# adamjorr/kbbq

Measured on AMD Instinct MI355X. Metric: recalibrated Gbases/sec, higher is better.
Workload: dtype u64

## Files before the change

kbbq_amd/csrc/engine.hip:

```cpp
#include <hip/hip_runtime.h>

#include <algorithm>
#include <cstdarg>
#include <cstdio>
#include <cstdlib>
#include <cstring>
#include <map>
#include <mutex>
#include <string>
#include <thread>
#include <vector>

#include "../../include/kbbq_engine.h"
#include "abi_internal.h"
#include "correct.h"
#include "correct_wave.h"
#include "device_common.h"
#include "host_model.h"

using namespace kbbq;

static thread_local char g_err[512] = "";
int kbbq_fail(int code, const char *fmt, ...) {
    va_list ap;
// ... 11 lines not shown
                        hipGetErrorString(_e), __FILE__, __LINE__);                                    \
    } while (0)

#include "kernels.h"
#include "bucket.h"
#include "long_reads.h"


struct FilterHost {
    FilterSpec spec;
    uint64_t *d_table = nullptr;
    uint64_t *d_patterns = nullptr;
    unsigned long long *d_inserted = nullptr;
    uint64_t table_bytes() const { return spec.n_blocks * kEngineBlockBytes; }
    FiltDev dev() const {
        FiltDev f;
        f.table = reinterpret_cast<ulonglong2 *>(d_table);
        f.patterns = reinterpret_cast<const ulonglong2 *>(d_patterns);
        f.n_blocks = spec.n_blocks;
        const ModMagic mm = make_mod_magic(spec.n_blocks);
        f.mod_magic = mm.m64;
        f.mod_m32 = mm.m32;
        f.salt0 = spec.salt[0];
        f.salt1 = spec.salt[1];
        return f;
    }
};

struct ProfileSlot {
    std::string name;
    uint64_t launches = 0;
    double ms = 0;
};
struct PendingEvent {
    int slot;
    hipEvent_t a, b;
};

struct Options {
    bool no_overlap = false;
    bool no_fastpath = false;
    bool lane_walk = false;
    bool no_pass4_pipeline = false;
    int pass2_side = 2;
    bool tally_general = false;
    bool infer_subset = true;
    bool debug_bucket = false;
    int bucket = -1;
    uint64_t bucket_records = 0;
    uint64_t pass4_piece = 0;
    int scan_blocks = -1;
    int walk_blocks = -1;
    int infer_blocks = 0;
};

struct kbbq_engine {
    kbbq_params p;
    Options opt;
    KParams K;
    hipStream_t stream = nullptr;
    hipStream_t stream2 = nullptr;
    hipEvent_t ev_main = nullptr, ev_side[2] = {nullptr, nullptr};
    hipEvent_t ev_draw = nullptr, ev_ins[2] = {nullptr, nullptr};
    bool ins_pending[2] = {false, false};
    int draw_turn = 0;
    bool side_busy[2] = {false, false};
    bool pass3_shared = false;
    unsigned long long *d_totals = nullptr;
    int side_turn = 0;
    uint32_t *d_qpresent = nullptr;
    uint32_t qpresent[8] = {};
    bool qpresent_known = false;
    uint8_t *d_dq_qslot = nullptr;
    int dq_slots = 0;
    uint32_t *d_rg_present[2] = {nullptr, nullptr};
    hipStream_t cur = nullptr;
    unsigned long long *cur_cnt = nullptr;
    FilterHost filt[2];
    Xoshiro256 seed_state;
    uint64_t draw_threshold = 0;
    bool draw_always = false;
    bool thresholds_set = false;
    std::vector<int32_t> thresholds;
    unsigned long long *d_hist = nullptr;
    uint64_t hist_cycle_words = 0, hist_dinuc_words = 0;
    DqTables dq;
    bool dq_set = false;
    int16_t *d_dq_base = nullptr;
    int8_t *d_dq_cycle = nullptr;
    int8_t *d_dq_dinuc = nullptr;
    void *scratch[24] = {};
    size_t scratch_bytes[24] = {};
    unsigned long long *d_counters = nullptr;
    unsigned int *d_tickets = nullptr;
    struct StageSlot {
        char *dev = nullptr;
        size_t bytes = 0;
        hipEvent_t h2d = nullptr, done[2] = {nullptr, nullptr};
        hipEvent_t d2h = nullptr;
        bool busy[2] = {false, false};
        bool d2h_pending = false;
        uint32_t gen = 0;
    } slot[3];
    int slot_turn = 0, cur_slot = -1;
    bool cur_slot_side = false;
    bool cur_h2d_recorded = false;
    bool async_call = false;
    uint64_t last_ticket = 0;
    hipStream_t copy = nullptr;
    uint64_t stats[4] = {0, 0, 0, 0};
    std::vector<ProfileSlot> prof;
    std::vector<PendingEvent> pending;
    uint32_t *d_qcum = nullptr, *d_errthr = nullptr;
    uint32_t qcum_len = 0;
    struct Buckets {
        int mode[2] = {-1, -1};
        bool allocated = false;
        uint64_t capacity = 0;
        void *l1 = nullptr, *l2 = nullptr;
        uint32_t *l1_cnt = nullptr, *l2_cnt = nullptr, *tickets = nullptr;
        unsigned long long *direct = nullptr;
        bool pending[2] = {false, false};
        double pending_est[2] = {0, 0};
        double frac_trusted = 0.75;
        double frac_used = 0.75;
        uint64_t bases_since[2] = {0, 0}, inserted_at_flush[2] = {0, 0};
        uint64_t flushes[2] = {0, 0};
        hipStream_t stream[2] = {nullptr, nullptr};
        hipEvent_t ev_flush = nullptr;
        unsigned long long *h_inserted = nullptr;
        hipEvent_t ev_est = nullptr;
        bool est_pending = false, est_known = false;
        uint64_t est_bases = 0, est_prev = 0, cur_bases = 0;
    } bk;
    hipEvent_t ev_infer = nullptr, ev_take[2] = {nullptr, nullptr};
    bool take_pending[2] = {false, false};
    int take_turn = 0;
    size_t attr_lds_tally = 0, attr_lds_recal = 0;
    std::map<const void *, size_t> attr_lds_correct;
};

namespace {

int ensure_scratch(kbbq_engine *e, int idx, size_t bytes) {
    if (e->scratch_bytes[idx] >= bytes) return KBBQ_OK;
    if (e->scratch[idx]) {
        HIP_TRY(hipStreamSynchronize(e->stream));
        HIP_TRY(hipStreamSynchronize(e->stream2));
        HIP_TRY(hipFree(e->scratch[idx]));
        e->scratch[idx] = nullptr;
        e->scratch_bytes[idx] = 0;
    }
    const size_t want = bytes + bytes / 8 + 256;
    HIP_TRY(hipMalloc(&e->scratch[idx], want));
    e->scratch_bytes[idx] = want;
    return KBBQ_OK;
}

static void plan_tally_slots(TallyPlan &P, const uint32_t mask[8], int max_slots, int n_rg) {
    memset(P.qslot, 255, sizeof P.qslot);
    memset(P.qof, 0, sizeof P.qof);
    P.n_slots = 0;
    max_slots = std::max(1, std::min(max_slots, 255));
    int top = -1, distinct = 0;
    for (int q = 0; q < KBBQ_NQ; ++q)
        if ((mask[q >> 5] >> (q & 31)) & 1) { top = q; ++distinct; }
    if (top >= 0 && top + 1 <= max_slots && (n_rg <= 1 || 2 * distinct >= top + 1)) {
        for (int q = 0; q <= top; ++q) { P.qof[q] = (uint8_t)q; P.qslot[q] = (uint8_t)q; }
        P.n_slots = top + 1;
        P.identity = 1;
    } else {
        for (int q = 0; q < KBBQ_NQ && P.n_slots < max_slots; ++q)
            if ((mask[q >> 5] >> (q & 31)) & 1) { P.qof[P.n_slots] = (uint8_t)q; P.qslot[q] = (uint8_t)P.n_slots++; }
        P.identity = 0;
    }
    if (P.n_slots == 0) { P.n_slots = 1; P.qof[0] = 0; P.qslot[0] = 0; P.identity = 1; }
    P.rg_base = 0; P.n_rgs = 1; P.cbase = 0; P.direct_cycles = 0;
}

struct Timed {
    kbbq_engine *e;
    int slot = -1;
    hipEvent_t a = nullptr, b = nullptr;
    hipStream_t on = nullptr;
    Timed(kbbq_engine *e_, const char *name, hipStream_t stream = nullptr) : e(e_), on(stream ? stream : e_->stream) {
        if (!(e->p.flags & KBBQ_F_PROFILE)) return;
        for (size_t i = 0; i < e->prof.size(); ++i)
            if (e->prof[i].name == name) slot = (int)i;
        if (slot < 0) {
            ProfileSlot s;
            s.name = name;
            e->prof.push_back(s);
            slot = (int)e->prof.size() - 1;
        }
        hipEventCreate(&a);
        hipEventCreate(&b);
        hipEventRecord(a, on);
    }
    ~Timed() {
        if (slot < 0) return;
        hipEventRecord(b, on);
        PendingEvent pe = {slot, a, b};
        e->pending.push_back(pe);
    }
};

void drain_profile(kbbq_engine *e) {
    for (size_t i = 0; i < e->pending.size(); ++i) {
        PendingEvent &pe = e->pending[i];
        float ms = 0;
        if (hipEventSynchronize(pe.b) == hipSuccess && hipEventElapsedTime(&ms, pe.a, pe.b) == hipSuccess) {
            e->prof[pe.slot].ms += ms;
            e->prof[pe.slot].launches += 1;
        }
        hipEventDestroy(pe.a);
        hipEventDestroy(pe.b);
    }
    e->pending.clear();
}

__global__ void k_add_counters(const unsigned long long *side, const unsigned long long *offcase, unsigned long long *totals) {
    totals[0] += side[0] + offcase[0];
    totals[1] += side[1];
}

int collect_totals(kbbq_engine *e) {
    unsigned long long t[2] = {0, 0};
    HIP_TRY(hipMemcpy(t, e->d_totals, 16, hipMemcpyDeviceToHost));
    e->stats[0] = t[0];
    e->stats[1] = t[1];
    e->side_busy[0] = e->side_busy[1] = false;
    return KBBQ_OK;
}

int sync_engine(kbbq_engine *e) {
    HIP_TRY(hipStreamSynchronize(e->stream));
    HIP_TRY(hipStreamSynchronize(e->stream2));
    if (e->side_busy[0] || e->side_busy[1]) {
        int rc = collect_totals(e);
        if (rc) return rc;
    }
    drain_profile(e);
    return KBBQ_OK;
}

struct HostBatchDone {
    kbbq_engine *e;
    HostBatchDone(kbbq_engine *e_, const kbbq_reads *) : e(e_) { e->cur_slot = -1; e->cur_slot_side = false; e->cur_h2d_recorded = false; e->last_ticket = 0; }
    ~HostBatchDone() {
        if (e->cur_slot < 0) return;
        kbbq_engine::StageSlot &s = e->slot[e->cur_slot];
        if (hipEventRecord(s.done[0], e->stream) == hipSuccess) s.busy[0] = true;
        if (e->cur_slot_side && hipEventRecord(s.done[1], e->stream2) == hipSuccess) s.busy[1] = true;
        if (e->async_call && e->cur_h2d_recorded) {
            e->last_ticket = ((uint64_t)s.gen << 8) | (uint64_t)(e->cur_slot + 1);
        } else if (e->cur_h2d_recorded) {
            hipEventSynchronize(s.h2d);
        } else {
            hipStreamSynchronize(e->copy);
        }
        e->cur_slot = -1;
    }
};

typedef KbbqDeviceGuard DeviceGuard;
#define ENGINE_DEVICE(e)                                                                              \
    if (!(e)) return fail(KBBQ_EINVAL, "null engine");                                                \
    DeviceGuard engine_device_guard((e)->p.device);                                                   \
    if (engine_device_guard.err != hipSuccess)                                                        \
        return fail(KBBQ_EIO, "hipSetDevice(%d): %s", (e)->p.device, hipGetErrorString(engine_device_guard.err))

hipStream_t shared_copy_stream(int device) {
    static std::mutex m;
    static std::map<int, hipStream_t> streams;
    std::lock_guard<std::mutex> lock(m);
    std::map<int, hipStream_t>::iterator it = streams.find(device);
    if (it != streams.end()) return it->second;
    hipStream_t st = nullptr;
    if (hipStreamCreateWithFlags(&st, hipStreamNonBlocking) != hipSuccess) return nullptr;
    streams[device] = st;
    return st;
}

int acquire_slot(kbbq_engine *e, size_t need, kbbq_engine::StageSlot **out) {
    kbbq_engine::StageSlot &s = e->slot[e->slot_turn];
    for (int t = 0; t < 2; ++t)
        if (s.busy[t]) { HIP_TRY(hipEventSynchronize(s.done[t])); s.busy[t] = false; }
    if (s.d2h_pending) { HIP_TRY(hipEventSynchronize(s.d2h)); s.d2h_pending = false; }
    s.gen += 1;
    if (s.bytes < need) {
// ... 328 lines not shown
    int rc = bucket_flush(e, 1 - w);
    if (rc) return rc;
    b.cur_bases = bases;
    if (b.pending[w] && b.pending_est[w] + est > 0.93 * (double)b.capacity) {
        if ((rc = bucket_flush(e, w, false))) return rc;
        if (w == 1) est = (est - 4096.0) / std::max(1e-9, b.frac_used) * b.frac_trusted + 4096.0;
    }
    b.cur_bases = 0;
    b.pending[w] = true;
    b.pending_est[w] += est;
    b.bases_since[w] += bases;
    return KBBQ_OK;
}

}


extern "C" {

const char *kbbq_last_error(void) { return g_err; }

int kbbq_engine_create(const kbbq_params *params, kbbq_engine **out) {
    if (!params || !out) return fail(KBBQ_EINVAL, "null argument");
    if (params->k < 1 || params->k > KBBQ_MAX_KMER) return fail(KBBQ_ERANGE, "k must be <= %d and > 0", KBBQ_MAX_KMER);
    if (params->n_rg < 1 || params->n_rg > 65535) return fail(KBBQ_EINVAL, "n_rg must be in 1..65535");
    if (params->max_read_len < 1 || params->max_read_len > KBBQ_MAX_READ_LEN)
        return fail(KBBQ_ERANGE, "max_read_len must be in 1..%d", KBBQ_MAX_READ_LEN);
    int ndev = 0;
    if (hipGetDeviceCount(&ndev) != hipSuccess || ndev == 0) return fail(KBBQ_ENODEV, "no HIP device visible");
    if (params->device < 0 || params->device >= ndev) return fail(KBBQ_ENODEV, "device %d of %d", params->device, ndev);
    DeviceGuard create_guard(params->device);
    HIP_TRY(create_guard.err);
    kbbq_engine *e = new kbbq_engine;
    e->p = *params;
    {
        Options &o = e->opt;
        auto env_set = [](const char *name) { const char *v = getenv(name); return v && *v; };
        auto env_int = [](const char *name, int dflt) { const char *v = getenv(name); return v && *v ? atoi(v) : dflt; };
        const int fl = params->flags;
        o.no_overlap = (fl & KBBQ_F_NO_OVERLAP) || env_set("KBBQ_NO_OVERLAP");
        o.no_fastpath = (fl & KBBQ_F_NO_FASTPATH) || env_set("KBBQ_NO_FASTPATH");
        o.lane_walk = (fl & KBBQ_F_LANE_WALK) || (getenv("KBBQ_CORRECT") && !strcmp(getenv("KBBQ_CORRECT"), "lane"));
        o.no_pass4_pipeline = (fl & KBBQ_F_NO_PASS4_PIPELINE) || env_set("KBBQ_NO_PASS4_PIPELINE");
        o.pass2_side = (fl & KBBQ_F_PASS2_INORDER) ? 0 : env_int("KBBQ_PASS2_SIDE", o.pass2_side);
        o.tally_general = env_set("KBBQ_TALLY_GENERAL");
        o.infer_subset = env_int("KBBQ_INFER_SUBSET", 1) != 0;
        o.debug_bucket = env_set("KBBQ_DEBUG_BUCKET");
        o.bucket = (fl & KBBQ_F_BUCKET_ON) ? 1 : (fl & KBBQ_F_BUCKET_OFF) ? 0 : env_set("KBBQ_BUCKET") ? (env_int("KBBQ_BUCKET", 0) != 0 ? 1 : 0) : -1;
        o.bucket_records = env_u64("KBBQ_BUCKET_RECORDS", 0);
        o.pass4_piece = env_u64("KBBQ_PASS4_PIECE", 0);
        o.scan_blocks = env_int("KBBQ_SCAN_BLOCKS", o.scan_blocks);
        o.walk_blocks = env_int("KBBQ_WALK_BLOCKS", o.walk_blocks);
        o.infer_blocks = env_int("KBBQ_INFER_BLOCKS", o.infer_blocks);
    }
    e->K.k = params->k;
    e->K.shift = 2u * (unsigned)(params->k - 1);
    e->K.mask = params->k < 32 ? ((1ULL << (2 * params->k)) - 1) : ~0ULL;
    e->K.nmask_bits = params->k < 32 ? ((1u << params->k) - 1) : 0xFFFFFFFFu;
    const double fprs[2] = {params->fpr_sampled, params->fpr_trusted};
    for (int w = 0; w < 2; ++w) {
        if (!make_filter_spec(params->approx_kmers, fprs[w], params->bloom_seed, e->filt[w].spec)) {
            delete e;
            return fail(KBBQ_EINVAL, "Error: Invalid bloom filter parameters. Adjust parameters and try again.");
        }
    }
    hipError_t he = hipStreamCreateWithFlags(&e->stream, hipStreamNonBlocking);
    if (he == hipSuccess) he = hipStreamCreateWithFlags(&e->stream2, hipStreamNonBlocking);
    if (he == hipSuccess) he = hipEventCreateWithFlags(&e->ev_main, hipEventDisableTiming);
    if (he == hipSuccess) he = hipEventCreateWithFlags(&e->ev_draw, hipEventDisableTiming);
    for (int t = 0; t < 2 && he == hipSuccess; ++t) he = hipEventCreateWithFlags(&e->ev_ins[t], hipEventDisableTiming);
    if (he == hipSuccess) he = hipEventCreateWithFlags(&e->ev_side[0], hipEventDisableTiming);
    if (he == hipSuccess) he = hipEventCreateWithFlags(&e->ev_side[1], hipEventDisableTiming);
    if (he == hipSuccess) he = hipStreamCreateWithFlags(&e->copy, hipStreamNonBlocking);
    if (he == hipSuccess) he = hipEventCreateWithFlags(&e->bk.ev_flush, hipEventDisableTiming);
    if (he == hipSuccess) he = hipEventCreateWithFlags(&e->bk.ev_est, hipEventDisableTiming);
    if (he == hipSuccess) he = hipEventCreateWithFlags(&e->ev_infer, hipEventDisableTiming);
    for (int t = 0; t < 2 && he == hipSuccess; ++t) he = hipEventCreateWithFlags(&e->ev_take[t], hipEventDisableTiming);
    if (he == hipSuccess) he = hipHostMalloc((void **)&e->bk.h_inserted, 64, hipHostMallocDefault);
    for (int i = 0; i < 3 && he == hipSuccess; ++i) {
        he = hipEventCreateWithFlags(&e->slot[i].h2d, hipEventDisableTiming);
        if (he == hipSuccess) he = hipEventCreateWithFlags(&e->slot[i].d2h, hipEventDisableTiming);
        for (int t = 0; t < 2 && he == hipSuccess; ++t) he = hipEventCreateWithFlags(&e->slot[i].done[t], hipEventDisableTiming);
    }
    e->cur = e->stream;
    if (he != hipSuccess) { kbbq_engine_destroy(e); return fail(KBBQ_EIO, "hipStreamCreate: %s", hipGetErrorString(he)); }
#define CREATE_TRY(expr)                                                                           \
    do {                                                                                           \
        hipError_t _e = (expr);                                                                    \
        if (_e != hipSuccess) {                                                                    \
            int code = _e == hipErrorOutOfMemory ? KBBQ_ENOMEM : KBBQ_EIO;                         \
            fail(code, "%s: %s", #expr, hipGetErrorString(_e));                                    \
            kbbq_engine_destroy(e);                                                                \
            return code;                                                                           \
        }                                                                                          \
    } while (0)
    CREATE_TRY(hipMalloc(&e->d_counters, 64));
    CREATE_TRY(hipMemset(e->d_counters, 0, 64));
    CREATE_TRY(hipMalloc(&e->d_tickets, 64));
    CREATE_TRY(hipMemset(e->d_tickets, 0, 64));
    CREATE_TRY(hipMalloc(&e->d_totals, 32));
    CREATE_TRY(hipMemset(e->d_totals, 0, 32));
    e->cur_cnt = e->d_counters;
    CREATE_TRY(hipMalloc(&e->d_dq_qslot, KBBQ_NQ));
    CREATE_TRY(hipMalloc(&e->d_qpresent, 32));
    for (int i = 0; i < 2; ++i) CREATE_TRY(hipMalloc(&e->d_rg_present[i], (((size_t)params->n_rg + 31) / 32) * 4 + 4));
    for (int w = 0; w < 2; ++w) {
        FilterHost &f = e->filt[w];
        CREATE_TRY(hipMalloc(&f.d_table, f.table_bytes()));
        CREATE_TRY(hipMalloc(&f.d_patterns, kNumPatterns * kEngineBlockBytes));
        CREATE_TRY(hipMalloc(&f.d_inserted, 8));
        std::vector<uint64_t> packed(kNumPatterns * 2);
        for (uint64_t i = 0; i < kNumPatterns; ++i) {
            if (!squeeze_block(&f.spec.patterns[i * 8], &packed[i * 2])) {
                kbbq_engine_destroy(e);
                return fail(KBBQ_ESTATE, "pattern %llu uses a bit outside the 128 the generator can reach", (unsigned long long)i);
            }
        }
        CREATE_TRY(hipMemcpy(f.d_patterns, packed.data(), kNumPatterns * kEngineBlockBytes, hipMemcpyHostToDevice));
    }
    e->hist_cycle_words = (uint64_t)params->n_rg * kNQ * 2 * params->max_read_len * 2;
    e->hist_dinuc_words = (uint64_t)params->n_rg * kNQ * 16 * 2;
    CREATE_TRY(hipMalloc(&e->d_hist, (e->hist_cycle_words + e->hist_dinuc_words) * 8));
    CREATE_TRY(hipMalloc(&e->d_dq_base, (size_t)params->n_rg * kNQ * 2));
    CREATE_TRY(hipMalloc(&e->d_dq_cycle, (size_t)params->n_rg * kNQ * 2 * params->max_read_len));
    CREATE_TRY(hipMalloc(&e->d_dq_dinuc, (size_t)params->n_rg * kNQ * 16));
    CREATE_TRY(hipMemcpyToSymbol(HIP_SYMBOL(c_jump), xoshiro_jump_table(), 64 * 4 * 8));
    e->seed_state.seed32(params->seed);
    e->draw_threshold = bernoulli_threshold(params->alpha, &e->draw_always);
    int rc = kbbq_engine_reset(e);
    if (rc) { kbbq_engine_destroy(e); return rc; }
    CREATE_TRY(hipDeviceSynchronize());
    *out = e;
    return KBBQ_OK;
}

void kbbq_engine_destroy(kbbq_engine *e) {
    if (!e) return;
    DeviceGuard destroy_guard(e->p.device);
    if (e->stream) { hipStreamSynchronize(e->stream); }
    if (e->stream2) hipStreamSynchronize(e->stream2);
    if (e->copy) hipStreamSynchronize(e->copy);
    drain_profile(e);
    for (int i = 0; i < 3; ++i) {
        hipFree(e->slot[i].dev);
        if (e->slot[i].h2d) hipEventDestroy(e->slot[i].h2d);
        if (e->slot[i].d2h) hipEventDestroy(e->slot[i].d2h);
        for (int t = 0; t < 2; ++t) if (e->slot[i].done[t]) hipEventDestroy(e->slot[i].done[t]);
    }
    if (e->copy) hipStreamDestroy(e->copy);
    if (e->bk.ev_flush) hipEventDestroy(e->bk.ev_flush);
    if (e->bk.ev_est) hipEventDestroy(e->bk.ev_est);
    if (e->ev_infer) hipEventDestroy(e->ev_infer);
    for (int t = 0; t < 2; ++t) if (e->ev_take[t]) hipEventDestroy(e->ev_take[t]);
    if (e->bk.h_inserted) hipHostFree(e->bk.h_inserted);
    for (int w = 0; w < 2; ++w) {
        hipFree(e->filt[w].d_table);
        hipFree(e->filt[w].d_patterns);
        hipFree(e->filt[w].d_inserted);
    }
    hipFree(e->d_hist);
    hipFree(e->d_dq_base);
    hipFree(e->d_dq_cycle);
    hipFree(e->d_dq_dinuc);
    hipFree(e->d_counters);
    hipFree(e->d_tickets);
    hipFree(e->d_totals);
    hipFree(e->d_dq_qslot);
    hipFree(e->d_qpresent);
    hipFree(e->d_rg_present[0]);
    hipFree(e->d_rg_present[1]);
    hipFree(e->d_qcum);
    hipFree(e->d_errthr);
    hipFree(e->bk.l1); hipFree(e->bk.l2); hipFree(e->bk.l1_cnt); hipFree(e->bk.l2_cnt); hipFree(e->bk.tickets); hipFree(e->bk.direct);
    for (int i = 0; i < 24; ++i) hipFree(e->scratch[i]);
    if (e->stream2) { hipStreamSynchronize(e->stream2); hipStreamDestroy(e->stream2); }
    if (e->ev_main) hipEventDestroy(e->ev_main);
    if (e->ev_draw) hipEventDestroy(e->ev_draw);
    for (int t = 0; t < 2; ++t) if (e->ev_ins[t]) hipEventDestroy(e->ev_ins[t]);
    for (int i = 0; i < 2; ++i) if (e->ev_side[i]) hipEventDestroy(e->ev_side[i]);
    if (e->stream) hipStreamDestroy(e->stream);
    delete e;
}

int kbbq_engine_reset(kbbq_engine *e) {
    ENGINE_DEVICE(e);
    if (!e) return fail(KBBQ_EINVAL, "null engine");
    int rc0 = sync_engine(e);
    if (rc0) return rc0;
    for (int w = 0; w < 2; ++w) {
        HIP_TRY(hipMemsetAsync(e->filt[w].d_table, 0, e->filt[w].table_bytes(), e->stream));
        HIP_TRY(hipMemsetAsync(e->filt[w].d_inserted, 0, 8, e->stream));
    }
    HIP_TRY(hipMemsetAsync(e->d_hist, 0, (e->hist_cycle_words + e->hist_dinuc_words) * 8, e->stream));
    HIP_TRY(hipMemsetAsync(e->d_counters, 0, 64, e->stream));
    HIP_TRY(hipMemsetAsync(e->d_totals, 0, 16, e->stream));
    HIP_TRY(hipMemsetAsync(e->d_qpresent, 0, 32, e->stream));
    memset(e->qpresent, 0, sizeof e->qpresent);
    e->qpresent_known = false;
    if (e->bk.allocated) {
        HIP_TRY(hipMemsetAsync(e->bk.l1_cnt, 0, kL1CntBytes, e->stream));
        HIP_TRY(hipMemsetAsync(e->bk.l2_cnt, 0, kL2CntBytes, e->stream));
        HIP_TRY(hipMemsetAsync(e->bk.direct, 0, 8, e->stream));
    }
    e->bk.est_pending = false;
    e->bk.est_known = false;
    e->bk.frac_trusted = 0.75;
    e->bk.stream[0] = e->bk.stream[1] = nullptr;
    for (int w = 0; w < 2; ++w) { e->bk.pending[w] = false; e->bk.pending_est[w] = 0; e->bk.bases_since[w] = 0; e->bk.inserted_at_flush[w] = 0; e->bk.flushes[w] = 0; }
    e->thresholds_set = false;
    e->dq_set = false;
    memset(e->stats, 0, sizeof e->stats);
    return sync_engine(e);
}

int kbbq_engine_sync(kbbq_engine *e) {
    ENGINE_DEVICE(e);
    { int frc = bucket_flush_all(e); if (frc) return frc; }
    if (!e) return fail(KBBQ_EINVAL, "null engine");
    return sync_engine(e);
}

void *kbbq_engine_stream(kbbq_engine *e) { return e ? (void *)e->stream : nullptr; }

int kbbq_engine_dims(kbbq_engine *e, uint64_t *n_rg, uint64_t *n_cycle) {
    if (!e) return fail(KBBQ_EINVAL, "null engine");
    if (n_rg) *n_rg = (uint64_t)e->p.n_rg;
    if (n_cycle) *n_cycle = (uint64_t)e->p.max_read_len;
    return KBBQ_OK;
}

int kbbq_engine_tune(kbbq_engine *e, const char *name, uint64_t value) {
    if (!e || !name) return fail(KBBQ_EINVAL, "null argument");
    if (!strcmp(name, "bucket_records")) {
        if (e->bk.allocated) return fail(KBBQ_ESTATE, "the record buffers are allocated already");
        e->opt.bucket_records = value;
    } else if (!strcmp(name, "pass4_piece")) {
        e->opt.pass4_piece = value;
    } else if (!strcmp(name, "scan_blocks") || !strcmp(name, "walk_blocks") || !strcmp(name, "infer_blocks")) {
        if (value > 17) return fail(KBBQ_EINVAL, "%s: 0 (as many as fit) to 16 workgroups per CU, 17 = default", name);
        (name[0] == 's' ? e->opt.scan_blocks : name[0] == 'w' ? e->opt.walk_blocks : e->opt.infer_blocks) = value == 17 ? (name[0] == 'i' ? 0 : -1) : (int)value;
    } else if (!strcmp(name, "infer_subset")) {
        e->opt.infer_subset = value != 0;
    } else if (!strcmp(name, "pass2_side")) {
        ENGINE_DEVICE(e);
        { int frc = bucket_flush_all(e); if (frc) return frc; }
        int rc = sync_engine(e);
        if (rc) return rc;
        if (value > 2) return fail(KBBQ_EINVAL, "pass2_side: 0, 1 or 2");
        e->opt.pass2_side = (int)value;
        e->bk.stream[0] = e->bk.stream[1] = nullptr;
    } else if (!strcmp(name, "no_overlap")) {
        ENGINE_DEVICE(e);
        { int frc = bucket_flush_all(e); if (frc) return frc; }
        int rc = sync_engine(e);
        if (rc) return rc;
        e->opt.no_overlap = value != 0;
        e->bk.stream[0] = e->bk.stream[1] = nullptr;
    } else {
        return fail(KBBQ_EINVAL, "unknown knob '%s'", name);
    }
    return KBBQ_OK;
}

int kbbq_filter_info_get(kbbq_engine *e, int which, kbbq_filter_info *out) {
    ENGINE_DEVICE(e);
    { int frc = bucket_flush_all(e); if (frc) return frc; }
    if (!e || !out || which < 0 || which > 1) return fail(KBBQ_EINVAL, "bad argument");
    const FilterSpec &s = e->filt[which].spec;
    memset(out, 0, sizeof *out);
    out->bits = s.bits;
    out->bits_unblocked = s.bits_unblocked;
    out->n_blocks = s.n_blocks;
    out->table_bytes = e->filt[which].table_bytes();
    out->random_seed = s.random_seed;
    out->n_hash = s.n_hash;
    out->n_salt = s.n_salt;
    for (uint32_t i = 0; i < s.n_salt; ++i) out->salt[i] = s.salt[i];
    int rc = sync_engine(e);
    if (rc) return rc;
    HIP_TRY(hipMemcpy(&out->inserted, e->filt[which].d_inserted, 8, hipMemcpyDeviceToHost));
    return KBBQ_OK;
}

void *kbbq_filter_device_table(kbbq_engine *e, int which) {
    if (!e || which < 0 || which > 1) return nullptr;
    DeviceGuard guard(e->p.device);
    if (guard.err != hipSuccess || bucket_flush_all(e) != KBBQ_OK) return nullptr;
    return e->filt[which].d_table;
}
void *kbbq_filter_device_counter(kbbq_engine *e, int which) { return e && which >= 0 && which < 2 ? e->filt[which].d_inserted : nullptr; }

int kbbq_filter_download(kbbq_engine *e, int which, uint64_t *host_words, uint64_t n_words) {
    ENGINE_DEVICE(e);
// ... 786 lines not shown
        const int dyn_len = ((max_len + 31) / 32) * 32;
        const size_t words = (size_t)C::words_for(dyn_len);
        const uint64_t fit = std::max<uint64_t>(1, ((uint64_t)1 << 30) / (words * 4 * BLOCK));
        const int blocks = (int)std::min<uint64_t>(std::min<uint64_t>((R.n_reads + BLOCK - 1) / BLOCK, 256 * 4), fit);
        const int slot = side ? 21 : 20;
        int rc = ensure_scratch(e, slot, (size_t)blocks * BLOCK * words * 4);
        if (rc) return rc;
        Timed t(e, "k_correct_long", e->cur);
        hipLaunchKernelGGL((k_correct<MAXL, BLOCK>), dim3(blocks), dim3(BLOCK), 0, e->cur, R, e->K, e->filt[1].dev(), list,
                           n_list, tmask, tw, err_bits, patch, e->cur_cnt, dyn_len, (uint32_t *)e->scratch[slot]);
        HIP_TRY(hipGetLastError());
        return KBBQ_OK;
    }
    const size_t lds = (size_t)C::WORDS * BLOCK * 4;
    size_t &raised = e->attr_lds_correct[(const void *)k_correct<MAXL, BLOCK>];
    if (lds > raised) {
        HIP_TRY(hipFuncSetAttribute((const void *)k_correct<MAXL, BLOCK>, hipFuncAttributeMaxDynamicSharedMemorySize, (int)lds));
        raised = lds;
    }
    Timed t(e, "k_correct", e->cur);
    const int blocks = (int)std::min<uint64_t>((R.n_reads + BLOCK - 1) / BLOCK, 256 * 8);
    hipLaunchKernelGGL((k_correct<MAXL, BLOCK>), dim3(blocks), dim3(BLOCK), lds, e->cur, R, e->K, e->filt[1].dev(), list,
                       n_list, tmask, tw, err_bits, patch, e->cur_cnt, 0, (uint32_t *)nullptr);
    HIP_TRY(hipGetLastError());
    return KBBQ_OK;
}

template <int NB, int NN>
static int launch_correct_wave(kbbq_engine *e, ReadsDev R, const uint32_t *list, const uint64_t *tmask, int tw,
                               uint32_t *err_bits, uint32_t *patch) {
    unsigned int *ticket = e->d_tickets + 3 + (e->cur_cnt != e->d_counters ? 1 : 0);
    HIP_TRY(hipMemsetAsync(ticket, 0, 4, e->cur));
    Timed t(e, "k_correct_wave", e->cur);
    const int blocks = wave_grid(R.n_reads, e->pass3_shared ? shared_cap(e, e->opt.walk_blocks, 2, NB <= 5 ? 160 : 512, !R.offsets) : 0);
    hipLaunchKernelGGL((k_correct_wave<NB, NN>), dim3(blocks), dim3(256), 0, e->cur, R, e->K, e->filt[1].dev(), list,
                       (const unsigned long long *)e->cur_cnt, tmask, tw, err_bits, patch, e->cur_cnt, ticket);
    HIP_TRY(hipGetLastError());
    return KBBQ_OK;
}
extern "C" {

static int build_read_index(kbbq_engine *e, const ReadsDev &R, int slot, hipStream_t stream, const uint32_t **index) {
    *index = nullptr;
    if (!R.offsets || !R.n_reads) return KBBQ_OK;
    const size_t entries = R.n_bases / READ_INDEX_STEP + 2;
    int rc = ensure_scratch(e, slot, entries * 4);
    if (rc) return rc;
    hipLaunchKernelGGL(k_read_index, dim3((unsigned)((R.n_reads + 255) / 256)), dim3(256), 0, stream, R.offsets, R.n_reads, (uint32_t *)e->scratch[slot]);
    HIP_TRY(hipGetLastError());
    *index = (const uint32_t *)e->scratch[slot];
    return KBBQ_OK;
}

static int run_tally(kbbq_engine *e, const ReadsDev &R, const uint32_t *err_bits, const uint32_t *patch, int max_len,
                     hipStream_t stream = nullptr) {
    if (!stream) stream = e->cur;
    HistDev H;
    H.cycle = e->d_hist;
    H.dinuc = e->d_hist + e->hist_cycle_words;
    H.n_rg = e->p.n_rg;
    H.n_cycle = e->p.max_read_len;
    const int n_rg = R.rg ? e->p.n_rg : 1;
    const int ccap = std::min(((max_len + 31) / 32) * 32, 192);
    if (!e->qpresent_known) {
        hipLaunchKernelGGL(k_qpresence, dim3(1024), dim3(256), 0, stream, R.qual, R.n_bases, e->d_qpresent);
        HIP_TRY(hipGetLastError());
        HIP_TRY(hipMemcpyAsync(e->qpresent, e->d_qpresent, 32, hipMemcpyDeviceToHost, stream));
        HIP_TRY(hipStreamSynchronize(stream));
    }
    const int n_windows = (max_len + ccap - 1) / ccap;
    const bool direct_cycles = n_windows > kTallyMaxWindows;
    const size_t per_slot = (direct_cycles ? 0 : (size_t)8 * ccap) + 128;
    TallyPlan P;
    plan_tally_slots(P, e->qpresent, (int)((152 * 1024 - 512) / per_slot), n_rg);
    P.direct_cycles = direct_cycles ? 1 : 0;
    const size_t per_rg = (size_t)P.n_slots * per_slot;
    const size_t budget = (size_t)n_rg * per_rg <= 70 * 1024 ? 70 * 1024 : 140 * 1024;
    const int per_launch = (int)std::max<size_t>(1, std::min<size_t>((size_t)n_rg, budget / per_rg));
    const size_t lds = (size_t)per_launch * per_rg + 4 + 256 + 4;
    if (lds > e->attr_lds_tally) {
        HIP_TRY(hipFuncSetAttribute((const void *)k_tally, hipFuncAttributeMaxDynamicSharedMemorySize, (int)lds));
        HIP_TRY(hipFuncSetAttribute((const void *)k_tally_uniform<true>, hipFuncAttributeMaxDynamicSharedMemorySize, (int)lds));
        HIP_TRY(hipFuncSetAttribute((const void *)k_tally_uniform<false>, hipFuncAttributeMaxDynamicSharedMemorySize, (int)lds));
        e->attr_lds_tally = lds;
    }
    const uint64_t groups = (R.n_bases + 15) / 16;
    const int blocks = (int)std::min<uint64_t>((groups + 1023) / 1024, lds <= 76 * 1024 ? 512 : 256);
    const int vec_ok = ((uintptr_t)R.qual & 15) == 0;
    const uint32_t *read_index;
    int rc = build_read_index(e, R, stream == e->stream2 ? 15 : 14, stream, &read_index);
    if (rc) return rc;
    const uint32_t *present = nullptr;
    if (n_rg > per_launch) {
        uint32_t *pr = e->d_rg_present[stream == e->stream2 ? 1 : 0];
        HIP_TRY(hipMemsetAsync(pr, 0, (((size_t)e->p.n_rg + 31) / 32) * 4, stream));
        hipLaunchKernelGGL(k_rg_presence, dim3((unsigned)((R.n_reads + 255) / 256)), dim3(256), 0, stream, R.rg, R.n_reads, (uint32_t)e->p.n_rg, pr);
        present = pr;
    }
    if (!e->opt.tally_general && !R.offsets && n_rg == 1 && n_windows == 1 && R.read_len >= 16 && (int)R.read_len <= ccap && R.n_bases < (1ULL << 32) && vec_ok &&
        e->p.n_rg == 1) {
        const unsigned long long inv_len = ~0ULL / R.read_len + 1;
        Timed t(e, "k_tally", stream);
        if (P.identity) hipLaunchKernelGGL(k_tally_uniform<false>, dim3(blocks), dim3(1024), lds, stream, R, H, err_bits, patch, ccap, 6, inv_len, P);
        else hipLaunchKernelGGL(k_tally_uniform<true>, dim3(blocks), dim3(1024), lds, stream, R, H, err_bits, patch, ccap, 6, inv_len, P);
        HIP_TRY(hipGetLastError());
        return KBBQ_OK;
    }
    Timed t(e, "k_tally", stream);
    for (int g = 0; g < n_rg; g += per_launch)
        for (int w = 0; w < (direct_cycles ? 1 : n_windows); ++w) {
            P.rg_base = g;
            P.n_rgs = std::min(per_launch, n_rg - g);
            P.cbase = w * ccap;
            hipLaunchKernelGGL(k_tally, dim3(blocks), dim3(1024), lds, stream, R, H, err_bits, patch, ccap, 6, vec_ok, P, present, read_index);
        }
    HIP_TRY(hipGetLastError());
    return KBBQ_OK;
}

int kbbq_errors_batch(kbbq_engine *e, const kbbq_reads *reads, uint64_t *errors_out) {
    ENGINE_DEVICE(e);
    { int frc = bucket_flush_all(e); if (frc) return frc; }
    if (!e || !reads) return fail(KBBQ_EINVAL, "null argument");
    const bool own_err = !(errors_out && reads->on_device);
    const bool overlap = own_err && !(errors_out && !reads->on_device) && !e->opt.no_overlap;
    int side = 0, rc;
    if (overlap) {
        side = e->side_turn;
        e->side_turn ^= 1;
        if (e->side_busy[side]) HIP_TRY(hipStreamWaitEvent(e->stream, e->ev_side[side], 0));
    } else {
        if ((rc = sync_engine(e))) return rc;
    }
    e->pass3_shared = overlap;
    HostBatchDone host_done(e, reads);
    ReadsDev R; int max_len;
    if ((rc = device_view(e, reads, &R, &max_len))) return rc;
    const bool long_reads = max_len > kStagedMax;
    const int NW = max_len <= 192 ? 3 : max_len <= 320 ? 5 : !long_reads ? 8 : 8 * ((std::max(1, max_len - e->p.k + 1) + 511) / 512);
    const int s_tmask = side ? 10 : 3, s_dirty = side ? 11 : 4, s_list = side ? 12 : 5, s_err = side ? 8 : 6, s_patch = side ? 9 : 7;
    if ((rc = ensure_scratch(e, s_tmask, R.n_reads * NW * 8))) return rc;
    if ((rc = ensure_scratch(e, s_dirty, R.n_reads))) return rc;
    if ((rc = ensure_scratch(e, s_list, R.n_reads * 4))) return rc;
    if ((rc = ensure_scratch(e, s_patch, R.n_reads * 4))) return rc;
    uint32_t *d_err;
    if (own_err) {
        if ((rc = ensure_scratch(e, s_err, (R.n_bases / 64 + 2) * 8))) return rc;
        d_err = (uint32_t *)e->scratch[s_err];
    } else {
        d_err = (uint32_t *)errors_out;
    }
    e->cur = e->stream;
    e->cur_cnt = e->d_counters + 4 * side;
    struct Restore { kbbq_engine *e; ~Restore() { e->cur = e->stream; e->cur_cnt = e->d_counters; } } restore = {e};
    HIP_TRY(hipMemsetAsync(d_err, 0, (R.n_bases / 64 + 1) * 8, e->cur));
    HIP_TRY(hipMemsetAsync(e->scratch[s_patch], 0, R.n_reads * 4, e->cur));
    HIP_TRY(hipMemsetAsync(e->cur_cnt, 0, 16, e->cur));
    uint64_t *tmask = (uint64_t *)e->scratch[s_tmask];
    uint8_t *dirty = (uint8_t *)e->scratch[s_dirty];
    uint32_t *list = (uint32_t *)e->scratch[s_list];
    uint32_t *patch = (uint32_t *)e->scratch[s_patch];
    const bool no_fast = e->opt.no_fastpath;
    if (long_reads) {
        Timed t(e, "k_scan_trusted_long", e->cur);
        hipLaunchKernelGGL(k_scan_trusted_long, dim3(wave_grid(R.n_reads)), dim3(256), 0, e->cur, R, e->K, e->filt[1].dev(), tmask, NW, dirty);
        HIP_TRY(hipGetLastError());
    } else if ((rc = dispatch_nw<LaunchScan>(max_len, e, R, tmask, dirty, d_err, (!no_fast && e->p.k >= 3) ? 1 : 0, max_len))) return rc;
    {
        Timed t(e, "k_compact", e->cur);
        hipLaunchKernelGGL(k_compact, dim3((unsigned)((R.n_reads + 1023) / 1024)), dim3(1024), 0, e->cur, dirty, R.n_reads, list, e->cur_cnt,
                           long_reads ? 0 : 1);
        HIP_TRY(hipGetLastError());
    }
    if (overlap) {
        HIP_TRY(hipEventRecord(e->ev_main, e->stream));
        HIP_TRY(hipStreamWaitEvent(e->stream2, e->ev_main, 0));
        e->cur = e->stream2;
        e->cur_slot_side = true;
    }
    const bool lane_form = e->opt.lane_walk;
    if (long_reads) {
        rc = launch_correct<0, 64>(e, R, list, e->cur_cnt, tmask, NW, d_err, patch, max_len, side);
    } else if (lane_form || e->p.k < 3) {
        if (max_len <= 160) rc = launch_correct<160, 256>(e, R, list, e->cur_cnt, tmask, NW, d_err, patch);
        else if (max_len <= 320) rc = launch_correct<320, 128>(e, R, list, e->cur_cnt, tmask, NW, d_err, patch);
        else rc = launch_correct<512, 64>(e, R, list, e->cur_cnt, tmask, NW, d_err, patch);
    } else {
        if (max_len <= 160) rc = launch_correct_wave<5, 3>(e, R, list, tmask, NW, d_err, patch);
        else if (max_len <= 320) rc = launch_correct_wave<10, 5>(e, R, list, tmask, NW, d_err, patch);
        else rc = launch_correct_wave<16, 8>(e, R, list, tmask, NW, d_err, patch);
    }
    if (rc) return rc;
    if (R.offcase && !long_reads) {
        if ((rc = ensure_scratch(e, side ? 18 : 17, R.n_reads * 4))) return rc;
        uint32_t *list3 = (uint32_t *)e->scratch[side ? 18 : 17];
        unsigned long long *cnt3 = e->d_counters + 6 + side;
        HIP_TRY(hipMemsetAsync(cnt3, 0, 8, e->cur));
        hipLaunchKernelGGL(k_compact, dim3((unsigned)((R.n_reads + 1023) / 1024)), dim3(1024), 0, e->cur, dirty, R.n_reads, list3, cnt3, 3);
        HIP_TRY(hipGetLastError());
        if (max_len <= 160) rc = launch_correct<160, 256>(e, R, list3, cnt3, tmask, NW, d_err, patch);
        else if (max_len <= 320) rc = launch_correct<320, 128>(e, R, list3, cnt3, tmask, NW, d_err, patch);
        else rc = launch_correct<512, 64>(e, R, list3, cnt3, tmask, NW, d_err, patch);
        if (rc) return rc;
    }
    if ((rc = run_tally(e, R, d_err, patch, max_len, e->cur))) return rc;
    if (!(R.offcase && !long_reads)) HIP_TRY(hipMemsetAsync(e->d_counters + 6 + side, 0, 8, e->cur));
    hipLaunchKernelGGL(k_add_counters, dim3(1), dim3(1), 0, e->cur, (const unsigned long long *)(e->d_counters + 4 * side),
                       (const unsigned long long *)(e->d_counters + 6 + side), e->d_totals);
    HIP_TRY(hipGetLastError());
    HIP_TRY(hipEventRecord(e->ev_side[side], e->cur));
    e->side_busy[side] = true;
    e->stats[2] += R.n_reads;
    if (!overlap) {
        if ((rc = sync_engine(e))) return rc;
        if (errors_out && !reads->on_device)
            HIP_TRY(hipMemcpy(errors_out, d_err, (R.n_bases / 64 + 1) * 8, hipMemcpyDeviceToHost));
    }
    return KBBQ_OK;
}

int kbbq_tally_batch(kbbq_engine *e, const kbbq_reads *reads, const uint64_t *errors) {
    ENGINE_DEVICE(e);
    { int frc = bucket_flush_all(e); if (frc) return frc; }
    if (!e || !errors) return fail(KBBQ_EINVAL, "null argument");
    HostBatchDone host_done(e, reads);
    ReadsDev R; int max_len;
    int rc = device_view(e, reads, &R, &max_len);
    if (rc) return rc;
    const uint32_t *d_err = (const uint32_t *)errors;
    if (!reads->on_device) {
        const size_t bytes = (reads->n_bases / 64 + 1) * 8;
        if ((rc = ensure_scratch(e, 16, bytes + 8))) return rc;
        HIP_TRY(hipMemsetAsync((char *)e->scratch[16] + bytes, 0, 8, e->stream));
        HIP_TRY(hipMemcpyAsync(e->scratch[16], errors, bytes, hipMemcpyHostToDevice, e->stream));
        d_err = (const uint32_t *)e->scratch[16];
    }
    if ((rc = run_tally(e, R, d_err, nullptr, max_len))) return rc;
    return reads->on_device ? KBBQ_OK : sync_engine(e);
}

void *kbbq_covariates_device(kbbq_engine *e, uint64_t *n_words) {
    if (!e) return nullptr;
    if (n_words) *n_words = e->hist_cycle_words + e->hist_dinuc_words;
    return e->d_hist;
}

static int fetch_hist(kbbq_engine *e, std::vector<uint64_t> &cyc, std::vector<uint64_t> &di) {
    int rc = sync_engine(e);
    if (rc) return rc;
    cyc.resize(e->hist_cycle_words);
    di.resize(e->hist_dinuc_words);
    HIP_TRY(hipMemcpy(cyc.data(), e->d_hist, e->hist_cycle_words * 8, hipMemcpyDeviceToHost));
    HIP_TRY(hipMemcpy(di.data(), e->d_hist + e->hist_cycle_words, e->hist_dinuc_words * 8, hipMemcpyDeviceToHost));
    return KBBQ_OK;
}

int kbbq_covariates_get(kbbq_engine *e, kbbq_covariates *out) {
    ENGINE_DEVICE(e);
// ... 408 lines not shown
```

kbbq_amd/csrc/kernels.h:

```cpp
#pragma once
#include <hip/hip_runtime.h>

#include "../../include/kbbq_engine.h"
#include "correct.h"
#include "correct_wave.h"
#include "device_common.h"

using namespace kbbq;


constexpr int DRAWS_PER_LANE = 4096;

__constant__ uint64_t c_jump[64][4];

__device__ __forceinline__ uint64_t xo_next(uint64_t (&s)[4]) {
    uint64_t x = s[1] * 5;
    x = (x << 7) | (x >> 57);
    x *= 9;
    const uint64_t t = s[1] << 17;
    s[2] ^= s[0];
    s[3] ^= s[1];
    s[1] ^= s[2];
    s[0] ^= s[3];
    s[2] ^= t;
// ... 886 lines not shown
                        count(lr, rg, q, second, cyc, (int)((ew >> i) & 1), cyc >= 1 && q >= minscore && !nn && !prev_n, (prev_b << 2) | b);
                    prev_b = b;
                    prev_n = nn;
                }
            }
            }
            starts += g0 != start ? 1 : 0;
        }
        {
            const int s = g0 < R.n_bases ? starts : 0;
            unsigned int tot = 0;
#pragma unroll
            for (int b = 0; b < 5; ++b) tot += (unsigned int)__popcll(__ballot((s >> b) & 1)) << b;
            if ((threadIdx.x & 63) == 0 && tot) atomicAdd(l_reads, tot);
        }
        __syncthreads();
        const bool flush = (direct ? (it & 0xFFFF) == 0xFFFF : *l_reads >= 40000u) || it + 1 == iters;
        __syncthreads();
        if (flush) {
            for (int lr = 0; lr < P.n_rgs; ++lr) {
                uint32_t *t = lds + lr * per_rg;
                const int rg = P.rg_base + lr;
                for (int w = threadIdx.x; w < cyc_words; w += blockDim.x) {
                    const uint32_t v = t[w], ve = t[cyc_words + w];
                    if (!v) continue;
                    t[w] = 0;
                    t[cyc_words + w] = 0;
                    for (int h = 0; h < 2; ++h) {
                        const uint32_t cnt = (v >> (16 * h)) & 0xFFFFu, cne = (ve >> (16 * h)) & 0xFFFFu;
                        if (!cnt) continue;
                        const int idx = 2 * w + h;
                        const int slot = idx % ccap, rest = idx / ccap;
                        const int q = P.qof[rest % ns], s = rest / ns;
                        const int c = cbase + (slot % (ccap >> 4)) * 16 + slot / (ccap >> 4);
                        if (c < H.n_cycle) {
                            atomicAdd(&H.cycle[cyc_index(H, rg, q, s, c) + 1], (unsigned long long)cnt);
                            if (cne) atomicAdd(&H.cycle[cyc_index(H, rg, q, s, c)], (unsigned long long)cne);
                        }
                    }
                }
                for (int w = threadIdx.x; w < ns * 16; w += blockDim.x) {
                    const uint32_t v = t[2 * cyc_words + w], ve = t[2 * cyc_words + ns * 16 + w];
                    const uint64_t cell = ((uint64_t)rg * KBBQ_NQ + P.qof[w >> 4]) * 16 + (w & 15);
                    if (v) { t[2 * cyc_words + w] = 0; atomicAdd(&H.dinuc[cell * 2 + 1], (unsigned long long)v); }
                    if (ve) { t[2 * cyc_words + ns * 16 + w] = 0; atomicAdd(&H.dinuc[cell * 2], (unsigned long long)ve); }
                }
            }
            if (threadIdx.x == 0) *l_reads = 0;
            __syncthreads();
        }
    }
}

template <bool MAP>
__global__ void __launch_bounds__(1024) k_tally_uniform(ReadsDev R, HistDev H, const uint32_t *err_bits, const uint32_t *patch,
                                                         int ccap, int minscore, unsigned long long inv_len, TallyPlan P) {
    extern __shared__ uint32_t lds[];
    const int ns = P.n_slots;
    const int L = (int)R.read_len;
    const int cyc_words = (2 * ccap * ns + 1) / 2, cstep = ccap >> 4;
    uint32_t *t_err = lds + cyc_words, *t_di = lds + 2 * cyc_words, *t_die = t_di + ns * 16;
    const int lds_words = 2 * cyc_words + 2 * ns * 16;
    uint8_t *l_qslot = reinterpret_cast<uint8_t *>(lds + lds_words);
    for (int i = threadIdx.x; i < lds_words; i += blockDim.x) lds[i] = 0;
    if (MAP && threadIdx.x < 256) l_qslot[threadIdx.x] = P.qslot[threadIdx.x];
    __syncthreads();
    auto count = [&](int second, int q, int cyc, int er, bool dinuc_ok, int d) {
        const int sl = MAP ? (int)l_qslot[q] : q;
        if (MAP ? sl != 255 : sl < ns) {
            const int idx = (second * ns + sl) * ccap + (cyc & 15) * cstep + (cyc >> 4);
            const uint32_t one = 1u << (16 * (idx & 1));
            atomicAdd(&lds[idx >> 1], one);
            if (er) atomicAdd(&t_err[idx >> 1], one);
            if (dinuc_ok) {
                atomicAdd(&t_di[sl * 16 + d], 1u);
                if (er) atomicAdd(&t_die[sl * 16 + d], 1u);
            }
        } else {
            atomicAdd(&H.cycle[cyc_index(H, 0, q, second, cyc) + 1], 1ULL);
            if (er) atomicAdd(&H.cycle[cyc_index(H, 0, q, second, cyc)], 1ULL);
            if (dinuc_ok) {
                atomicAdd(&H.dinuc[((uint64_t)q * 16 + d) * 2 + 1], 1ULL);
                if (er) atomicAdd(&H.dinuc[((uint64_t)q * 16 + d) * 2], 1ULL);
            }
        }
    };
    auto flush = [&]() {
        for (int w = threadIdx.x; w < cyc_words; w += blockDim.x) {
            const uint32_t v = lds[w], ve = t_err[w];
            if (!v) continue;
            lds[w] = 0;
            t_err[w] = 0;
            for (int h = 0; h < 2; ++h) {
                const uint32_t cnt = (v >> (16 * h)) & 0xFFFFu, cne = (ve >> (16 * h)) & 0xFFFFu;
                if (!cnt) continue;
                const int idx = 2 * w + h;
                const int slot = idx % ccap, rest = idx / ccap;
                const int q = MAP ? (int)P.qof[rest % ns] : rest % ns, sec = rest / ns;
                const int c = (slot % cstep) * 16 + slot / cstep;
                if (c < H.n_cycle) {
                    atomicAdd(&H.cycle[cyc_index(H, 0, q, sec, c) + 1], (unsigned long long)cnt);
                    if (cne) atomicAdd(&H.cycle[cyc_index(H, 0, q, sec, c)], (unsigned long long)cne);
                }
            }
        }
        for (int w = threadIdx.x; w < ns * 16; w += blockDim.x) {
            const uint32_t v = t_di[w], ve = t_die[w];
            const uint64_t cell = (uint64_t)(MAP ? (int)P.qof[w >> 4] : (w >> 4)) * 16 + (w & 15);
// ... 310 lines not shown
```

Baseline: 22.72.

## Run uniform tally on a third stream with smaller workgroups to overlap correction

Adds a third HIP stream so the uniform-shape tally kernel for a batch runs concurrently with the next batch's scan and correction work. The stream is gated by events, and the error and patch scratch buffers are now triple-buffered. The tally kernel is templated on thread count, and the side-stream launch uses 256- or 512-thread workgroups with at most 256 blocks so it leaves CUs free for the concurrent walk kernels. This adds cross-stream event bookkeeping and buffer rotation, which risks ordering bugs and extra scheduling overhead.

```diff
diff --git a/kbbq_amd/csrc/engine.hip b/kbbq_amd/csrc/engine.hip
--- a/kbbq_amd/csrc/engine.hip
+++ b/kbbq_amd/csrc/engine.hip
@@ -87,6 +87,8 @@
     int scan_blocks = -1;
     int walk_blocks = -1;
     int infer_blocks = 0;
+    int tally_stream = 0;
+    int tally_threads = 256;
 };
 
 struct kbbq_engine {
@@ -96,6 +98,11 @@
     hipStream_t stream = nullptr;
     hipStream_t stream2 = nullptr;
     hipEvent_t ev_main = nullptr, ev_side[2] = {nullptr, nullptr};
+    hipStream_t stream3 = nullptr;
+    hipEvent_t ev_walk[2] = {nullptr, nullptr}, ev_tally[3] = {nullptr, nullptr, nullptr};
+    bool tally_busy[3] = {false, false, false};
+    bool set_by_side[2] = {false, false};
+    int tally_turn = 0;
     hipEvent_t ev_draw = nullptr, ev_ins[2] = {nullptr, nullptr};
     bool ins_pending[2] = {false, false};
     int draw_turn = 0;
@@ -182,6 +189,7 @@
     if (e->scratch[idx]) {
         HIP_TRY(hipStreamSynchronize(e->stream));
         HIP_TRY(hipStreamSynchronize(e->stream2));
+        if (e->stream3) HIP_TRY(hipStreamSynchronize(e->stream3));
         HIP_TRY(hipFree(e->scratch[idx]));
         e->scratch[idx] = nullptr;
         e->scratch_bytes[idx] = 0;
@@ -265,12 +273,17 @@
     e->stats[0] = t[0];
     e->stats[1] = t[1];
     e->side_busy[0] = e->side_busy[1] = false;
+    e->set_by_side[0] = e->set_by_side[1] = false;
     return KBBQ_OK;
 }
 
 int sync_engine(kbbq_engine *e) {
     HIP_TRY(hipStreamSynchronize(e->stream));
     HIP_TRY(hipStreamSynchronize(e->stream2));
+    if (e->stream3) {
+        HIP_TRY(hipStreamSynchronize(e->stream3));
+        e->tally_busy[0] = e->tally_busy[1] = e->tally_busy[2] = false;
+    }
     if (e->side_busy[0] || e->side_busy[1]) {
         int rc = collect_totals(e);
         if (rc) return rc;
@@ -705,6 +718,9 @@
         o.scan_blocks = env_int("KBBQ_SCAN_BLOCKS", o.scan_blocks);
         o.walk_blocks = env_int("KBBQ_WALK_BLOCKS", o.walk_blocks);
         o.infer_blocks = env_int("KBBQ_INFER_BLOCKS", o.infer_blocks);
+        o.tally_stream = env_int("KBBQ_TALLY_STREAM", o.tally_stream);
+        if (o.tally_stream < -1 || o.tally_stream > 1) o.tally_stream = Options().tally_stream;
+        o.tally_threads = env_int("KBBQ_TALLY_THREADS", o.tally_threads) == 512 ? 512 : 256;
     }
     e->K.k = params->k;
     e->K.shift = 2u * (unsigned)(params->k - 1);
@@ -792,6 +808,7 @@
     DeviceGuard destroy_guard(e->p.device);
     if (e->stream) { hipStreamSynchronize(e->stream); }
     if (e->stream2) hipStreamSynchronize(e->stream2);
+    if (e->stream3) hipStreamSynchronize(e->stream3);
     if (e->copy) hipStreamSynchronize(e->copy);
     drain_profile(e);
     for (int i = 0; i < 3; ++i) {
@@ -827,6 +844,9 @@
     hipFree(e->bk.l1); hipFree(e->bk.l2); hipFree(e->bk.l1_cnt); hipFree(e->bk.l2_cnt); hipFree(e->bk.tickets); hipFree(e->bk.direct);
     for (int i = 0; i < 24; ++i) hipFree(e->scratch[i]);
     if (e->stream2) { hipStreamSynchronize(e->stream2); hipStreamDestroy(e->stream2); }
+    if (e->stream3) { hipStreamSynchronize(e->stream3); hipStreamDestroy(e->stream3); }
+    for (int i = 0; i < 2; ++i) if (e->ev_walk[i]) hipEventDestroy(e->ev_walk[i]);
+    for (int i = 0; i < 3; ++i) if (e->ev_tally[i]) hipEventDestroy(e->ev_tally[i]);
     if (e->ev_main) hipEventDestroy(e->ev_main);
     if (e->ev_draw) hipEventDestroy(e->ev_draw);
     for (int t = 0; t < 2; ++t) if (e->ev_ins[t]) hipEventDestroy(e->ev_ins[t]);
@@ -892,6 +912,12 @@
     } else if (!strcmp(name, "scan_blocks") || !strcmp(name, "walk_blocks") || !strcmp(name, "infer_blocks")) {
         if (value > 17) return fail(KBBQ_EINVAL, "%s: 0 (as many as fit) to 16 workgroups per CU, 17 = default", name);
         (name[0] == 's' ? e->opt.scan_blocks : name[0] == 'w' ? e->opt.walk_blocks : e->opt.infer_blocks) = value == 17 ? (name[0] == 'i' ? 0 : -1) : (int)value;
+    } else if (!strcmp(name, "tally_stream")) {
+        if (value > 1 && value != ~(uint64_t)0) return fail(KBBQ_EINVAL, "tally_stream: 0 (side stream), 1 (third stream) or -1 (default)");
+        e->opt.tally_stream = value == ~(uint64_t)0 ? -1 : (int)value;
+    } else if (!strcmp(name, "tally_threads")) {
+        if (value != 0 && value != 256 && value != 512) return fail(KBBQ_EINVAL, "tally_threads: 256 or 512, 0 = default");
+        e->opt.tally_threads = value ? (int)value : 256;
     } else if (!strcmp(name, "infer_subset")) {
         e->opt.infer_subset = value != 0;
     } else if (!strcmp(name, "pass2_side")) {
@@ -1784,8 +1810,13 @@
     return KBBQ_OK;
 }
 
+static bool tally_uniform_shape(const kbbq_engine *e, const kbbq_reads *in) {
+    return !e->opt.tally_general && !in->offsets && e->p.n_rg == 1 && in->read_len >= 16 && in->read_len <= 192 &&
+           in->n_bases < (1ULL << 32) && ((uintptr_t)in->qual & 15) == 0;
+}
+
 static int run_tally(kbbq_engine *e, const ReadsDev &R, const uint32_t *err_bits, const uint32_t *patch, int max_len,
-                     hipStream_t stream = nullptr) {
+                     hipStream_t stream = nullptr, int small_wg = 0) {
     if (!stream) stream = e->cur;
     HistDev H;
     H.cycle = e->d_hist;
@@ -1814,6 +1845,10 @@
         HIP_TRY(hipFuncSetAttribute((const void *)k_tally, hipFuncAttributeMaxDynamicSharedMemorySize, (int)lds));
         HIP_TRY(hipFuncSetAttribute((const void *)k_tally_uniform<true>, hipFuncAttributeMaxDynamicSharedMemorySize, (int)lds));
         HIP_TRY(hipFuncSetAttribute((const void *)k_tally_uniform<false>, hipFuncAttributeMaxDynamicSharedMemorySize, (int)lds));
+        HIP_TRY(hipFuncSetAttribute((const void *)k_tally_uniform<true, 256>, hipFuncAttributeMaxDynamicSharedMemorySize, (int)lds));
+        HIP_TRY(hipFuncSetAttribute((const void *)k_tally_uniform<false, 256>, hipFuncAttributeMaxDynamicSharedMemorySize, (int)lds));
+        HIP_TRY(hipFuncSetAttribute((const void *)k_tally_uniform<true, 512>, hipFuncAttributeMaxDynamicSharedMemorySize, (int)lds));
+        HIP_TRY(hipFuncSetAttribute((const void *)k_tally_uniform<false, 512>, hipFuncAttributeMaxDynamicSharedMemorySize, (int)lds));
         e->attr_lds_tally = lds;
     }
     const uint64_t groups = (R.n_bases + 15) / 16;
@@ -1833,8 +1868,16 @@
         e->p.n_rg == 1) {
         const unsigned long long inv_len = ~0ULL / R.read_len + 1;
         Timed t(e, "k_tally", stream);
-        if (P.identity) hipLaunchKernelGGL(k_tally_uniform<false>, dim3(blocks), dim3(1024), lds, stream, R, H, err_bits, patch, ccap, 6, inv_len, P);
-        else hipLaunchKernelGGL(k_tally_uniform<true>, dim3(blocks), dim3(1024), lds, stream, R, H, err_bits, patch, ccap, 6, inv_len, P);
+        const int small_blocks = (int)std::min<uint64_t>((groups + small_wg - 1) / std::max(small_wg, 1), 256);
+#define KBBQ_TALLY_UNIFORM(MAP)                                                                                                        \
+    do {                                                                                                                              \
+        if (small_wg == 256) hipLaunchKernelGGL((k_tally_uniform<MAP, 256>), dim3(small_blocks), dim3(256), lds, stream, R, H, err_bits, patch, ccap, 6, inv_len, P);       \
+        else if (small_wg == 512) hipLaunchKernelGGL((k_tally_uniform<MAP, 512>), dim3(small_blocks), dim3(512), lds, stream, R, H, err_bits, patch, ccap, 6, inv_len, P); \
+        else hipLaunchKernelGGL((k_tally_uniform<MAP>), dim3(blocks), dim3(1024), lds, stream, R, H, err_bits, patch, ccap, 6, inv_len, P);                                    \
+    } while (0)
+        if (P.identity) KBBQ_TALLY_UNIFORM(false);
+        else KBBQ_TALLY_UNIFORM(true);
+#undef KBBQ_TALLY_UNIFORM
         HIP_TRY(hipGetLastError());
         return KBBQ_OK;
     }
@@ -1857,10 +1900,35 @@
     const bool own_err = !(errors_out && reads->on_device);
     const bool overlap = own_err && !(errors_out && !reads->on_device) && !e->opt.no_overlap;
     int side = 0, rc;
+    bool third = false;
+    if (overlap && reads->on_device && e->opt.tally_stream != 0 && tally_uniform_shape(e, reads)) {
+        const int len = (int)reads->read_len;
+        const bool wave_walk = !e->opt.lane_walk && e->p.k >= 3;
+        third = e->opt.tally_stream == 1 ||
+                (shared_cap(e, e->opt.scan_blocks, 4, len) > 0 && wave_walk && shared_cap(e, e->opt.walk_blocks, 2, len <= 160 ? 160 : 512) > 0);
+    }
+    int set = 0;
     if (overlap) {
         side = e->side_turn;
         e->side_turn ^= 1;
         if (e->side_busy[side]) HIP_TRY(hipStreamWaitEvent(e->stream, e->ev_side[side], 0));
+        set = side;
+        if (third) {
+            if (!e->stream3) {
+                HIP_TRY(hipStreamCreateWithFlags(&e->stream3, hipStreamNonBlocking));
+                for (int i = 0; i < 2; ++i) HIP_TRY(hipEventCreateWithFlags(&e->ev_walk[i], hipEventDisableTiming));
+                for (int i = 0; i < 3; ++i) HIP_TRY(hipEventCreateWithFlags(&e->ev_tally[i], hipEventDisableTiming));
+            }
+            set = e->tally_turn;
+            e->tally_turn = (e->tally_turn + 1) % 3;
+            if (set < 2 && e->set_by_side[set]) {
+                if (set != side) HIP_TRY(hipStreamWaitEvent(e->stream, e->ev_side[set], 0));
+                e->set_by_side[set] = false;
+            }
+        } else {
+            e->set_by_side[side] = true;
+        }
+        if (e->tally_busy[set]) HIP_TRY(hipStreamWaitEvent(e->stream, e->ev_tally[set], 0));
     } else {
         if ((rc = sync_engine(e))) return rc;
     }
@@ -1870,7 +1938,8 @@
     if ((rc = device_view(e, reads, &R, &max_len))) return rc;
     const bool long_reads = max_len > kStagedMax;
     const int NW = max_len <= 192 ? 3 : max_len <= 320 ? 5 : !long_reads ? 8 : 8 * ((std::max(1, max_len - e->p.k + 1) + 511) / 512);
-    const int s_tmask = side ? 10 : 3, s_dirty = side ? 11 : 4, s_list = side ? 12 : 5, s_err = side ? 8 : 6, s_patch = side ? 9 : 7;
+    const int s_tmask = side ? 10 : 3, s_dirty = side ? 11 : 4, s_list = side ? 12 : 5;
+    const int s_err = set == 2 ? 19 : set ? 8 : 6, s_patch = set == 2 ? 23 : set ? 9 : 7;
     if ((rc = ensure_scratch(e, s_tmask, R.n_reads * NW * 8))) return rc;
     if ((rc = ensure_scratch(e, s_dirty, R.n_reads))) return rc;
     if ((rc = ensure_scratch(e, s_list, R.n_reads * 4))) return rc;
@@ -1935,7 +2004,13 @@
         else rc = launch_correct<512, 64>(e, R, list3, cnt3, tmask, NW, d_err, patch);
         if (rc) return rc;
     }
-    if ((rc = run_tally(e, R, d_err, patch, max_len, e->cur))) return rc;
+    if (third) {
+        HIP_TRY(hipEventRecord(e->ev_walk[side], e->cur));
+        HIP_TRY(hipStreamWaitEvent(e->stream3, e->ev_walk[side], 0));
+        if ((rc = run_tally(e, R, d_err, patch, max_len, e->stream3, e->opt.tally_threads))) return rc;
+        HIP_TRY(hipEventRecord(e->ev_tally[set], e->stream3));
+        e->tally_busy[set] = true;
+    } else if ((rc = run_tally(e, R, d_err, patch, max_len, e->cur))) return rc;
     if (!(R.offcase && !long_reads)) HIP_TRY(hipMemsetAsync(e->d_counters + 6 + side, 0, 8, e->cur));
     hipLaunchKernelGGL(k_add_counters, dim3(1), dim3(1), 0, e->cur, (const unsigned long long *)(e->d_counters + 4 * side),
                        (const unsigned long long *)(e->d_counters + 6 + side), e->d_totals);
diff --git a/kbbq_amd/csrc/kernels.h b/kbbq_amd/csrc/kernels.h
--- a/kbbq_amd/csrc/kernels.h
+++ b/kbbq_amd/csrc/kernels.h
@@ -962,8 +962,8 @@
     }
 }
 
-template <bool MAP>
-__global__ void __launch_bounds__(1024) k_tally_uniform(ReadsDev R, HistDev H, const uint32_t *err_bits, const uint32_t *patch,
+template <bool MAP, int THREADS = 1024>
+__global__ void __launch_bounds__(THREADS) k_tally_uniform(ReadsDev R, HistDev H, const uint32_t *err_bits, const uint32_t *patch,
                                                          int ccap, int minscore, unsigned long long inv_len, TallyPlan P) {
     extern __shared__ uint32_t lds[];
     const int ns = P.n_slots;
```

New measurement: 22.67, median of 2. Within noise of the previous version (-0.2%).
